# marbl/MHAP

Measured on AMD Instinct MI355X. Metric: overlaps/sec, higher is better.
Workload: dtype int64

## Files before the change

### include/mhap_hip.h

```cpp
#ifndef MHAP_HIP_H
#define MHAP_HIP_H

#include <stddef.h>
#include <stdint.h>

#ifdef __cplusplus
extern "C" {
#endif

#define MHAP_OK 0
#define MHAP_E_INVALID (-1)
#define MHAP_E_HIP (-2)
#define MHAP_E_NOMEM (-3)
#define MHAP_E_STATE (-4)
#define MHAP_E_IO (-5)

#define MHAP_STRAND_OK 0
#define MHAP_STRAND_ZERO_NGRAMS 1
#define MHAP_STRAND_TOO_SHORT 2

typedef struct mhap_params {
  int32_t kmer_size;
  int32_t num_hashes;
  int32_t ordered_kmer_size;
// ... 180 lines not shown

int mhap_align_pairs_banded(mhap_handle* h, const uint8_t* bases, int64_t n_bases, const int64_t* pairs , int64_t n,
                            int32_t* results );

int mhap_realign_plan(const mhap_record* recs, int64_t n, const int64_t* read_ids, const int64_t* offsets, const int32_t* lengths,
                      int64_t n_reads, double max_shift, int32_t band , int64_t* pairs );
const char* mhap_realign_plan_error(void);

int mhap_realign_records(mhap_handle* h, const uint8_t* bases, int64_t n_bases, const int64_t* read_ids, const int64_t* offsets,
                         const int32_t* lengths, int64_t n_reads, const mhap_record* recs, int64_t n, int32_t band,
                         mhap_record* out, int32_t* detail );

int mhap_pair_kmer_stats(mhap_handle* h, const uint8_t* bases, int64_t n_bases, const int64_t* pairs, int64_t n, int32_t k,
                         int32_t bottom_k, const uint8_t* skip, int64_t n_skip, int32_t* out, int32_t* paths);
void* mhap_ksim_dev_create(mhap_handle* h);
void mhap_ksim_dev_destroy(void* dev);
int mhap_ksim_dev_pair_stats(void* dev, const uint8_t* bases, int64_t n_bases, const int64_t* pairs, int64_t n, int32_t k, int32_t bottom_k,
                             const uint8_t* skip, int64_t n_skip, int32_t* out, int32_t* paths);
int mhap_ksim_dev_trials(void* dev, uint64_t seed, int64_t trial0, int64_t n, int32_t length, int32_t offset, double error_rate,
                         double ins_pct, double del_pct, double sub_pct, int32_t flags, const uint8_t* ref_bases,
                         const int64_t* ref_offsets, const int32_t* ref_lengths, int64_t n_ref, int32_t k, int32_t bottom_k,
                         const uint8_t* skip, int64_t n_skip, int32_t* stats, uint8_t* reads, int32_t* meta, int32_t* events,
                         int64_t* failed_trial);
int mhap_pair_kmer_stats_paths(const int64_t* pairs, int64_t n, int32_t k, int64_t lds_bytes, int32_t hashed, int32_t* path);

#define MHAP_KSIM_ONE_SIDED 1
#define MHAP_KSIM_SIM_ONLY 2
void* mhap_ksim_create(int64_t seed, int32_t length, int32_t offset, double error_rate, double ins_pct, double del_pct, double sub_pct,
                       int32_t flags, const uint8_t* ref_bases, const int64_t* ref_offsets, const int32_t* ref_lengths, int64_t n_ref);
int64_t mhap_ksim_next(void* state, int64_t n_trials, uint8_t* reads, int32_t* meta);
const char* mhap_ksim_error(void* state, int32_t* role);
void mhap_ksim_destroy(void* state);

int mhap_synth_reads(uint64_t seed, int64_t n, int32_t len, double coverage, double error_rate, char* bases);
int mhap_synth_reads_shard(uint64_t seed, int64_t n, int32_t len, double coverage, double error_rate, int64_t shard,
                           int64_t nshards, char* bases);
int mhap_synth_reads_repeats(uint64_t seed, int64_t n, int32_t len, double coverage, double error_rate, int64_t shard,
                             int64_t nshards, int32_t rep_len, int32_t rep_spacing, double rep_div, char* bases);
int mhap_synth_reads_genome(uint64_t seed, const uint8_t* genome, int64_t G, int64_t n, const int32_t* lengths, const int64_t* offsets,
                            double error_rate, char* bases);

int mhap_synth_truth(uint64_t seed, int64_t n, int32_t len, double coverage, int64_t G, const int32_t* lengths, double error_rate,
                     int64_t shard, int64_t nshards, int64_t* start, int64_t* span, int8_t* strand, int32_t* n_ins, int32_t* n_del,
                     int32_t* n_sub);

int mhap_histogram_stats(const int32_t* vals, const int64_t* numbers, int64_t n, double percent, double* mean, double* stdev, int64_t* cut);

int mhap_hash_kmer(const char* kmer, int32_t len, int32_t do_rc, int64_t* out);

int mhap_selftest_hash_windows(const char* seq, int32_t len, int32_t k, int32_t k2, int64_t* out64, int32_t* out32);
int mhap_selftest_bloom(const int64_t* hashes, int64_t n, int64_t size_bloom, const int64_t* probes, int64_t np, uint8_t* out_flags,
                        int64_t* out2);
int mhap_selftest_transpose32(uint32_t* a32);
int mhap_selftest_pass_min(int32_t S, int32_t k2, double threshold, double* scores, int32_t* pass_min);
int mhap_selftest_xorshift_jump(uint64_t key, int32_t nsteps, uint64_t* out);
int mhap_selftest_xorshift_unjump(uint64_t x, int32_t nsteps, uint64_t* out);
int mhap_selftest_kmer_windows(const char* seq, int32_t len, int32_t k, int32_t canonical, uint64_t* out, uint8_t* valid);
int mhap_selftest_overlap_lane(const int32_t* A, int32_t nA, int32_t lenA, const int32_t* B, int32_t nB, int32_t lenB,
                               double max_shift, int32_t stride, int32_t* out8);

#ifdef __cplusplus
}
#endif
#endif
```

### mhap_amd/api.py

```python
import ctypes as C
import os

import numpy as np

_HERE = os.path.dirname(os.path.abspath(__file__))
_LIB_PATH = os.environ.get("MHAP_LIB_PATH") or os.path.join(_HERE, "lib", "libmhaphip.so")
_lib = None

KERNEL_NAMES = ["hash_kmers", "kmer_weight", "minhash", "ordered", "candidate", "overlap", "index_build", "index_query"]


class MhapError(RuntimeError):
    """MhapRuntimeException analogue (J/impl/MhapRuntimeException.java:32)."""


class _Params(C.Structure):
    _fields_ = [("kmer_size", C.c_int32), ("num_hashes", C.c_int32), ("ordered_kmer_size", C.c_int32),
                ("ordered_sketch_size", C.c_int32), ("num_min_matches", C.c_int32), ("min_store_length", C.c_int32),
                ("min_olap_length", C.c_int32), ("device", C.c_int32), ("threshold", C.c_double),
                ("max_shift", C.c_double), ("repeat_weight", C.c_double)]


class _Stats(C.Structure):
    _fields_ = [("strands_indexed", C.c_int64), ("queries_searched", C.c_int64), ("candidates_compared", C.c_int64),
                ("matches_found", C.c_int64), ("slot_compares", C.c_int64), ("table_elements", C.c_int64),
                ("slow_pairs", C.c_int64), ("index_splits", C.c_int64)]


class _KTimes(C.Structure):
    _fields_ = [("ms", C.c_double * 8), ("launches", C.c_int64 * 8)]


class _Fasta(C.Structure):
    _fields_ = [("bases", C.c_void_p), ("offsets", C.c_void_p), ("lengths", C.c_void_p), ("ids", C.c_void_p),
                ("n", C.c_int64), ("total_bases", C.c_int64), ("headers", C.c_void_p), ("headers_bytes", C.c_int64)]


RECORD_DTYPE = np.dtype([("from_id", "<i8"), ("to_id", "<i8"), ("score", "<f8"), ("raw", "<f8"), ("a1", "<i4"),
                         ("a2", "<i4"), ("alen", "<i4"), ("b1", "<i4"), ("b2", "<i4"), ("blen", "<i4"),
                         ("to_rc", "<i4"), ("pad", "<i4")])
_SINK = C.CFUNCTYPE(C.c_int, C.c_void_p, C.c_int64, C.c_void_p)
_GATE = C.CFUNCTYPE(C.c_int, C.c_void_p)

EXPORTED_SYMBOLS = [
    "mhap_create", "mhap_destroy", "mhap_last_error", "mhap_default_params", "mhap_set_filter", "mhap_index_add_reads",
    "mhap_sketch_batch", "mhap_index_add_sketches", "mhap_index_size", "mhap_index_export", "mhap_index_clear", "mhap_index_prepare",
    "mhap_sketch_reads_device", "mhap_index_set_device", "mhap_find_matches_self", "mhap_find_matches_reads",
    "mhap_get_stats", "mhap_get_kernel_times", "mhap_reset_kernel_times", "mhap_set_stream", "mhap_synchronize",
    "mhap_format_record", "mhap_fasta_read", "mhap_fasta_free", "mhap_synth_reads", "mhap_hash_kmer",
    "mhap_selftest_hash_windows", "mhap_selftest_overlap_lane", "mhap_stage_reads", "mhap_index_add_staged",
    "mhap_sketch_staged_device", "mhap_find_matches_self_shard", "mhap_synth_reads_shard", "mhap_selftest_transpose32", "mhap_selftest_pass_min", "mhap_selftest_xorshift_jump", "mhap_selftest_xorshift_unjump", "mhap_find_matches_sketches",
    "mhap_synth_reads_repeats", "mhap_synth_reads_genome", "mhap_find_matches_device", "mhap_set_filter_whitelist", "mhap_set_filter_file", "mhap_selftest_bloom", "mhap_set_second_stage_gate",
    "mhap_dist_unique_id", "mhap_dist_init", "mhap_dist_finalize", "mhap_dist_find_matches_self", "mhap_dist_find_matches_reads", "mhap_dist_last_timing", "mhap_dist_exchange_timing", "mhap_dist_info", "mhap_dist_selftest", "mhap_dist_set_eager", "mhap_dist_eager_searches",
    "mhap_group_create", "mhap_group_destroy", "mhap_group_size", "mhap_group_rank", "mhap_group_last_error", "mhap_group_add_reads", "mhap_group_clear",
    "mhap_group_find_matches_self", "mhap_group_find_matches_reads", "mhap_group_get_stats", "mhap_abi_version", "mhap_abi_sizes",
    "mhap_index_reserve", "mhap_fasta_scan_open", "mhap_fasta_scan_free", "mhap_fasta_scan_reads", "mhap_fasta_scan_bases", "mhap_fasta_scan_info",
    "mhap_index_add_scan", "mhap_find_matches_scan", "mhap_group_add_scan",
    "mhap_kmer_count_begin", "mhap_kmer_count_add_reads", "mhap_kmer_count_add_scan", "mhap_kmer_count_finish", "mhap_kmer_counts_info",
    "mhap_kmer_counts_lines", "mhap_kmer_counts_write", "mhap_kmer_counts_free", "mhap_selftest_kmer_windows",
    "mhap_kmer_count_finish_flags", "mhap_kmer_counts_histogram_size", "mhap_kmer_counts_histogram", "mhap_kmer_counts_write_histogram",
    "mhap_histogram_stats",
    "mhap_synth_truth", "mhap_align_pairs",
    "mhap_align_pairs_banded", "mhap_realign_plan", "mhap_realign_plan_error", "mhap_realign_records",
    "mhap_pair_kmer_stats", "mhap_pair_kmer_stats_paths", "mhap_ksim_create", "mhap_ksim_next", "mhap_ksim_error", "mhap_ksim_destroy",
    "mhap_ksim_dev_create", "mhap_ksim_dev_destroy", "mhap_ksim_dev_pair_stats", "mhap_ksim_dev_trials",
]
MHAP_KMER_HISTOGRAM = 1
ABI_VERSION = 3


def load_library(build_if_missing=True):
    global _lib
    if _lib is not None:
        return _lib
    if not os.path.exists(_LIB_PATH):
        if not build_if_missing:
            raise MhapError(f"{_LIB_PATH} is missing: run `python -m mhap_amd.build`")
        from . import build as _b
        _b.build()
    try:
        import torch
    except Exception:
        pass
    try:
        lib = C.CDLL(_LIB_PATH)
    except OSError as e:
        raise MhapError(f"cannot load the HIP extension {_LIB_PATH}: {e}") from e
    lib.mhap_last_error.restype = C.c_char_p
    lib.mhap_last_error.argtypes = [C.c_void_p]
    lib.mhap_destroy.restype = None
    lib.mhap_destroy.argtypes = [C.c_void_p]
    lib.mhap_fasta_free.restype = None
    lib.mhap_default_params.restype = None
    lib.mhap_group_destroy.restype = None
    lib.mhap_group_destroy.argtypes = [C.c_void_p]
    lib.mhap_group_rank.restype = C.c_void_p
    lib.mhap_group_rank.argtypes = [C.c_void_p, C.c_int32]
    lib.mhap_group_last_error.restype = C.c_char_p
    lib.mhap_group_last_error.argtypes = [C.c_void_p]
    lib.mhap_group_size.argtypes = [C.c_void_p]
    lib.mhap_fasta_scan_free.restype = None
    lib.mhap_fasta_scan_free.argtypes = [C.c_void_p]
    lib.mhap_fasta_scan_reads.restype = C.c_int64
    lib.mhap_fasta_scan_reads.argtypes = [C.c_void_p]
    lib.mhap_fasta_scan_bases.restype = C.c_int64
    lib.mhap_fasta_scan_bases.argtypes = [C.c_void_p]
    lib.mhap_kmer_counts_free.restype = None
    lib.mhap_kmer_counts_free.argtypes = [C.c_void_p]
    for name, nargs in (("mhap_kmer_counts_info", 4), ("mhap_kmer_counts_lines", 2), ("mhap_kmer_counts_write", 1),
                        ("mhap_kmer_counts_histogram_size", 1), ("mhap_kmer_counts_histogram", 2), ("mhap_kmer_counts_write_histogram", 1)):
        getattr(lib, name).argtypes = [C.c_void_p] + [C.c_void_p] * nargs
    lib.mhap_histogram_stats.argtypes = [C.c_void_p, C.c_void_p, C.c_int64, C.c_double, C.c_void_p, C.c_void_p, C.c_void_p]
    lib.mhap_ksim_create.restype = C.c_void_p
    lib.mhap_ksim_create.argtypes = [C.c_int64, C.c_int32, C.c_int32, C.c_double, C.c_double, C.c_double, C.c_double, C.c_int32,
                                     C.c_void_p, C.c_void_p, C.c_void_p, C.c_int64]
    lib.mhap_ksim_next.restype = C.c_int64
    lib.mhap_ksim_next.argtypes = [C.c_void_p, C.c_int64, C.c_void_p, C.c_void_p]
    lib.mhap_ksim_error.restype = C.c_char_p
# ... 888 lines not shown
```

### mhap_amd/csrc/kernels.hpp

```cpp
#pragma once
#include "device_common.hpp"

namespace mhap {

constexpr int HASH_TILE = 1024;
constexpr int WEIGHT_THREADS = 1024;
constexpr int WEIGHT_MAXIT = 24;
constexpr int MH_U = 4;
constexpr int ORD_THREADS = 256;
constexpr int ORD_BINS = 2048;
constexpr int CAND_TQ = 128;
constexpr int CAND_TM = 128;
constexpr int CAND_KS = 32;
constexpr int OVL_THREADS = 128;
#ifndef MH_INV_CT
#define MH_INV_CT 2048
#endif
constexpr int INV_CT = MH_INV_CT;

constexpr int BS_WCLASSES = 6;
constexpr int BS_WMAX = 32;
struct StrandInfo { int32_t valid; int32_t mode; int32_t cnt[BS_WCLASSES + 1]; int32_t pad; };

struct FilterTable {
  const int64_t* keys;
  const double* vals;
  uint32_t mask;
  uint32_t size;
  int32_t enabled;
  int32_t no_tf;
  double range;
  const unsigned long long* bloom; uint64_t bloom_bits; int32_t bloom_k; int32_t bloom_mode;
};

constexpr int META_W = 4;

struct Candidate { int32_t q; int32_t m; };

struct DevRecord { int32_t q, m; double score; int32_t raw, a1, a2, b1, b2, pad; };

struct SearchParams {
  int32_t H, S, k2;
  int32_t num_min_matches, min_store_length;
  int32_t to_self;
  int32_t own_queries;
  double max_shift, threshold;
};

void launch_hash_kmers(hipStream_t st, const ReadDesc* descs, int64_t nstrands, int max_len, const uint8_t* store, int64_t* keys,
                       int32_t* h32, int k, int k2, const uint64_t* luts, int only_mat);
void build_kmer_hash_luts(uint64_t* out);
int weight_grid(int num_cus, int64_t nstrands, int max_len, int k);
bool strand_hashes_from_codes(int length, int k, int k2);
void launch_kmer_weights(hipStream_t st, int num_cus, const ReadDesc* descs, int64_t nstrands, int max_len, const int64_t* keys,
                         uint32_t* wts, uint32_t* perm, uint32_t* slabs, int64_t slab_entries, unsigned long long* counter, int k,
                         const FilterTable& ft, double repeat_weight, StrandInfo* info, bool fused, const uint8_t* store,
                         const uint64_t* luts, const int32_t* order, int32_t* slist);
bool launch_minhash(hipStream_t st, hipStream_t st_weighted, int nblocks, int64_t n_unweighted, int64_t n_weighted, const ReadDesc* descs, int64_t nstrands, const int64_t* keys, const uint32_t* wts,
                    const uint32_t* perm, const StrandInfo* info, const uint8_t* store, const uint64_t* luts, int k, int k2, int H,
                    unsigned long long* counter, int32_t* out_rows, int64_t out_stride, int32_t* out_status, int64_t status_stride,
                    const uint64_t* jump, int jump_na, const int32_t* slist, uint32_t* qbuf, const uint64_t* unjump, const uint64_t* jump_w1, unsigned long long* merge,
                    int max_nk);
size_t minhash_merge_bytes(int nblocks, int H);
void build_xorshift_unjump_tables(int na, int nq, uint64_t* out);
int minhash_wgs_per_cu(int H);
size_t minhash_queue_bytes(int nblocks_total, int H);
int minhash_queue_words(int H);
constexpr int XS_JUMP_LOG2 = 2;
constexpr int XS_JUMP_NQ = BS_WMAX;
#ifndef MH_W1_JUMP_NA
#define MH_W1_JUMP_NA 16
#endif
constexpr int W1_JUMP_NA = MH_W1_JUMP_NA;
inline int w1_jump_tables(int H) { return W1_JUMP_NA + ((H + 1) >> XS_JUMP_LOG2) / W1_JUMP_NA + 1; }
void build_xorshift_jump_tables(int na, int nq, uint64_t* out);
void launch_fix_status(hipStream_t st, int32_t* meta, int64_t nreads);
size_t ordered_lds_bytes(int cap, int code_words, int stage_wide);
void launch_ordered(hipStream_t st, const ReadDesc* descs, int64_t nstrands, int max_len_codes, int max_len, const int32_t* h32,
                    const uint8_t* store, const uint64_t* luts, int k2, int S, int cap, int32_t* out_rows, int64_t out_stride,
                    int32_t* out_meta, int64_t meta_stride, int64_t first = 0, int64_t count = -1);

void launch_candidates(hipStream_t st, const int32_t* minhash, int64_t row_stride, const int32_t* qminhash, int64_t qrow_stride,
                       const int32_t* qlist, int nq, int ne, const int64_t* ids, const int64_t* qids, const int32_t* meta,
                       const int32_t* qmeta, const SearchParams& sp, const long long* rowstart, long long nblocks_tri, Candidate* cand,
                       unsigned long long* cand_count, unsigned long long cand_cap);
constexpr int MHAP_MAX_NUM_HASHES = 8192;
int minhash_waves_per_workgroup(int H);
struct InvIndex {
  uint32_t* ends;
  uint2* items;
  uint32_t nb, shift;
  uint64_t slot_stride;
  uint32_t ne;
  uint32_t grouped;
  uint32_t group_t, class_log;
  uint32_t* lines;
  uint32_t nl_log, line_lb, line_ebits;
  uint32_t tile_entries, tiles;
  uint2* staged;
  uint32_t* tile_counts;
  uint32_t* bin_start;
  uint32_t* bin_long;
};
void launch_query_iota(hipStream_t st, int32_t* qlist, int first, int n);
int index_tile_entries(int ne);
void index_group_params(int64_t entries, InvIndex& ix);
int index_coarse_bins();
bool index_line_params(int64_t entries, uint32_t nb, uint32_t& nl_log, uint32_t& lb, uint32_t& ebits);
size_t index_line_bytes(int H, uint32_t nl_log);
int index_max_buckets_log();
void launch_index_verify(hipStream_t st, const int32_t* minhash, int64_t row_stride, const int32_t* meta, int ne, int H, const InvIndex& ix,
                         unsigned long long* missing);
bool launch_index_build(hipStream_t st, const int32_t* minhash, int64_t row_stride, const int32_t* meta, int ne, int H, const InvIndex& ix);
void launch_index_query(hipStream_t st, const InvIndex& ix, const int32_t* qminhash, int64_t qrow_stride,
                        const int32_t* qlist, int nq, const int64_t* ids, const int64_t* qids, const int32_t* meta, const int32_t* qmeta,
                        const SearchParams& sp, Candidate* cand, unsigned long long* cand_count, unsigned long long cand_cap,
                        unsigned long long* split_count, unsigned long long* elements_total, int32_t* big, unsigned long long* big_count, int tier,
                        unsigned long long* elements_spread);
int index_elements_spread_words();
int index_query_dense_ranges(int64_t entries);
bool index_query_tiers();
bool index_query_tier_ok(int tier, int64_t entries, int num_min_matches);
void oj_stats_dump();
void launch_overlap(hipStream_t st, int nblocks, const Candidate* cand, const unsigned long long* cand_count, unsigned long long cand_cap,
                    const int32_t* ordered, int64_t ord_stride, const int32_t* meta, const int32_t* qordered, int64_t qord_stride,
                    const int32_t* qmeta, const SearchParams& sp, const double* score_table, int32_t* scratch, int64_t scratch_per_lane,
                    DevRecord* recs, unsigned long long* rec_count, unsigned long long rec_cap, unsigned long long* compared, int spread);
size_t overlap_join_wide_lds_bytes(int S, int shape);
int overlap_join_wide_blocks_per_cu(int S, int shape);
int overlap_join_wide_waves_per_block(int shape);
// ... 31 lines not shown
```

### mhap_amd/csrc/mhap_capi.hip

```cpp
#include <algorithm>
#include <atomic>
#include <cmath>
#include <cstdio>
#include <cstdlib>
#include <chrono>
#include <cstring>
#include <condition_variable>
#include <functional>
#include <mutex>
#include <string>
#include <thread>
#include <vector>

#include "../../include/mhap_hip.h"
static double hp_now() { return std::chrono::duration<double, std::milli>(std::chrono::steady_clock::now().time_since_epoch()).count(); }
#define HPROF(tag) do { if (getenv("MHAP_HOST_PROF")) fprintf(stderr, "[host] %-28s %.3f ms\n", tag, hp_now()); } while (0)
#define DBGSYNC(h, tag) do { if (getenv("MHAP_DEBUG_SYNC")) { fprintf(stderr, "[dbg] %s launched\n", tag); hipError_t _e = hipStreamSynchronize((h)->stream); fprintf(stderr, "[dbg] %s done: %s\n", tag, hipGetErrorString(_e)); } } while (0)
#include "kernels.hpp"
#include "mhap_internal.hpp"
#include "overlap_lane.hpp"

using namespace mhap;

namespace {
// ... 1633 lines not shown
    for (int i = 0; i < 8; i++) y ^= T[i * 256 + (int)((x >> (8 * i)) & 255u)];
    x = y;
  }
  for (int t = 0; t < r; t++) x = xorshift_step(x);
  *out = x;
  return MHAP_OK;
}

int mhap_selftest_xorshift_unjump(uint64_t x, int32_t nsteps, uint64_t* out) {
  if (!out || nsteps < 1 || nsteps > (1 << 15)) return MHAP_E_INVALID;
  int a = (nsteps + (1 << XS_JUMP_LOG2) - 1) >> XS_JUMP_LOG2;
  const int r = (a << XS_JUMP_LOG2) - nsteps;
  const int qa = a > W1_JUMP_NA ? (a - 1) / W1_JUMP_NA : 0;
  a -= qa * W1_JUMP_NA;
  std::vector<uint64_t> ut((size_t)(W1_JUMP_NA + qa) * 2048);
  build_xorshift_unjump_tables(W1_JUMP_NA, qa, ut.data());
  uint64_t y = x;
  if (qa > 0) {
    const uint64_t* T = ut.data() + (size_t)(W1_JUMP_NA + qa - 1) * 2048;
    uint64_t z = 0;
    for (int i = 0; i < 8; i++) z ^= T[i * 256 + (int)((y >> (8 * i)) & 255u)];
    y = z;
  }
  {
    const uint64_t* T = ut.data() + (size_t)(a - 1) * 2048;
    uint64_t z = 0;
    for (int i = 0; i < 8; i++) z ^= T[i * 256 + (int)((y >> (8 * i)) & 255u)];
    y = z;
  }
  for (int t = 0; t < r; t++) y = xorshift_step(y);
  *out = y;
  return MHAP_OK;
}

int mhap_selftest_bloom(const int64_t* hashes, int64_t n, int64_t size_bloom, const int64_t* probes, int64_t np, uint8_t* out_flags, int64_t* out2) {
  if ((n > 0 && !hashes) || (np > 0 && (!probes || !out_flags)) || !out2) return MHAP_E_INVALID;
  std::vector<unsigned long long> words; uint64_t bit_size = 0; int k = 0;
  build_bloom(hashes, n, size_bloom, words, bit_size, k);
  for (int64_t i = 0; i < np; i++) out_flags[i] = bloom_might_contain(words.data(), bit_size, k, (uint64_t)probes[i]) ? 1 : 0;
  out2[0] = (int64_t)bit_size; out2[1] = k;
  return MHAP_OK;
}

int mhap_selftest_pass_min(int32_t S, int32_t k2, double threshold, double* scores, int32_t* pass_min) {
  if (S < 1 || S > 8192 || k2 < 1 || !pass_min) return MHAP_E_INVALID;
  std::vector<double> tbl; std::vector<int32_t> pm;
  fill_score_table(S, k2, tbl);
  build_pass_min(tbl, S, threshold, pm);
  if (scores) memcpy(scores, tbl.data(), tbl.size() * 8);
  memcpy(pass_min, pm.data(), pm.size() * 4);
  return MHAP_OK;
}

int mhap_selftest_transpose32(uint32_t* a32) {
  if (!a32) return MHAP_E_INVALID;
  uint32_t a[32];
  memcpy(a, a32, sizeof a);
  transpose32(a);
  memcpy(a32, a, sizeof a);
  return MHAP_OK;
}

int mhap_selftest_overlap_lane(const int32_t* A, int32_t nA, int32_t lenA, const int32_t* B, int32_t nB, int32_t lenB, double max_shift,
                               int32_t stride, int32_t* out8) {
  if (!A || !B || !out8 || stride < 1) return MHAP_E_INVALID;
  const int maxrec = 2 * std::max(nA, nB) + 2;
  std::vector<int32_t> scratch((size_t)3 * (size_t)maxrec * (size_t)stride, 0);
  LaneScratch sc; sc.base = scratch.data(); sc.stride = stride; sc.maxrec = maxrec;
  PlainView va{A, nA}, vb{B, nB};
  const LaneOverlap r = lane_overlap(va, lenA, vb, lenB, max_shift, sc);
  out8[0] = r.empty; out8[1] = r.valid; out8[2] = r.a1; out8[3] = r.a2; out8[4] = r.b1; out8[5] = r.b2; out8[6] = r.inter; out8[7] = r.kk;
  return MHAP_OK;
}

}

namespace mhap {
int internal_find_matches_device(mhap_handle* h, const void* d_q_minhash, const void* d_q_ordered, const void* d_q_meta, const int64_t* ids,
                                 const int64_t* d_ids_dev, int64_t m, int to_self, mhap_record_sink sink, void* user) {
  return find_matches_device_impl(h, d_q_minhash, d_q_ordered, d_q_meta, ids, d_ids_dev, m, to_self, sink, user);
}
}
```

### mhap_amd/csrc/sketch_kernels.hip

```cpp
#include <cstdlib>
#include <cstring>

#include "kernels.hpp"
#include <algorithm>

namespace mhap {

constexpr int HASH_SEG = 4096;
constexpr int HASH_LUT_WORDS = 3 * 256;

void build_kmer_hash_luts(uint64_t* out) {
  const uint64_t c1 = 0x87c37b91114253d5ULL, c2 = 0x4cf5ad432745937fULL;
  const uint32_t d1 = 0xcc9e2d51U, d2 = 0x1b873593U;
  const char* acgt = "ACGT";
  for (int idx = 0; idx < 256; idx++) {
    uint64_t block = 0;
    for (int c = 0; c < 4; c++) block |= (uint64_t)(uint8_t)acgt[(idx >> (2 * c)) & 3] << (16 * c);
    uint64_t k1 = block * c1; k1 = rotl64(k1, 31); k1 *= c2;
    uint64_t k2 = block * c2; k2 = rotl64(k2, 33); k2 *= c1;
    uint32_t a = (uint32_t)block, b = (uint32_t)(block >> 32);
    a *= d1; a = rotl32(a, 15); a *= d2;
    b *= d1; b = rotl32(b, 15); b *= d2;
    out[idx] = k1; out[256 + idx] = k2; out[512 + idx] = (uint64_t)a | ((uint64_t)b << 32);
  }
// ... 1792 lines not shown
      if (a.n_tail > 0) (void)hipMemsetAsync(merge, 0xFF, (size_t)a.n_tail * (size_t)H * 8, st);
      a.prof = nullptr;
      if (profmode) {
        static unsigned long long* dprof1 = nullptr;
        if (!dprof1) (void)hipMalloc(&dprof1, 8 * sizeof(unsigned long long));
        (void)hipMemsetAsync(dprof1, 0, 8 * sizeof(unsigned long long), st);
        a.prof = dprof1;
        static hipEvent_t pe0 = nullptr, pe1 = nullptr;
        if (!pe0) { (void)hipEventCreate(&pe0); (void)hipEventCreate(&pe1); }
        (void)hipEventRecord(pe0, st);
        if (qcap == BS_QCAP) hipLaunchKernelGGL((minhash_w1_kernel<true, true>), dim3(nb), dim3(256), lds1, st, a);
        else hipLaunchKernelGGL((minhash_w1_kernel<true, false>), dim3(nb), dim3(256), lds1, st, a);
        (void)hipEventRecord(pe1, st);
        unsigned long long hp[8];
        (void)hipMemcpyAsync(hp, dprof1, sizeof(hp), hipMemcpyDeviceToHost, st);
        (void)hipStreamSynchronize(st);
        const double tot = (double)hp[7];
        float pms = 0.f; (void)hipEventElapsedTime(&pms, pe0, pe1);
        fprintf(stderr, "[minhash w1 prof] launch %.3f ms, %d waves: mean shader clock %.0f MHz (wave-clocks / waves / time)\n", pms, nb * 4,
                pms > 0.f ? tot / ((double)nb * 4.0) / ((double)pms * 1e3) : 0.0);
        fprintf(stderr, "[minhash w1 prof] rows %llu (first-type %llu)  wave-clocks: total %.3g  key load+transpose %.1f%%  first-row slots %.1f%% (%.0f clocks/step)  "
                        "later-row slots %.1f%% (%.0f clocks/step)  drains %.1f%%  candidates/row %.0f\n", hp[4], hp[5], tot, 100.0 * hp[0] / tot, 100.0 * hp[1] / tot,
                hp[5] ? (double)hp[1] / ((double)hp[5] * H) : 0.0, 100.0 * hp[2] / tot, hp[4] > hp[5] ? (double)hp[2] / ((double)(hp[4] - hp[5]) * H) : 0.0,
                100.0 * hp[3] / tot, hp[4] ? (double)hp[6] / (double)hp[4] : 0.0);
      } else
        if (qcap == BS_QCAP) hipLaunchKernelGGL((minhash_w1_kernel<false, true>), dim3(nb), dim3(256), lds1, st, a);
        else hipLaunchKernelGGL((minhash_w1_kernel<false, false>), dim3(nb), dim3(256), lds1, st, a);
      if (a.n_tail > 0)
        hipLaunchKernelGGL(minhash_w1_finish_kernel, dim3((unsigned)((a.n_tail * (long long)H + 255) / 256)), dim3(256), 0, st, a);
      if (witness) snprintf(w1_path, sizeof(w1_path), "w1 n_whole %lld n_tail %lld rmax %d stagger %d", (long long)a.n_whole, (long long)a.n_tail, a.rmax, a.stagger);
    }
    if (witness)
      fprintf(stderr, "[minhash] strands %lld weight-1 %lld weighted %lld nblocks %d: weight-1 launch %s; weighted launch %s\n", (long long)nstrands,
              (long long)n_unweighted, (long long)n_weighted, nblocks, w1_path, nb_w > 0 ? (split ? "split" : "wave") : "none");
    return nb_w > 0;
  }
}


#ifdef MH_ORD_PROF
__device__ unsigned long long g_ord_prof[8];
#define ORD_TICK(k) do { __syncthreads(); if (threadIdx.x == 0) { const unsigned long long t_ = wall_clock64(); atomicAdd(&g_ord_prof[k], t_ - ord_t0); ord_t0 = t_; } } while (0)
#else
#define ORD_TICK(k) do { } while (0)
#endif
__device__ __forceinline__ uint32_t mm3_mul5c(uint32_t h) {
  uint32_t t;
  asm("v_lshl_add_u32 %0, %1, 2, %1" : "=v"(t) : "v"(h));
  return t + 0xe6546b64U;
}
constexpr uint32_t ORD_BUCKET_MAX = 32;
__device__ inline uint64_t okey(int32_t h, int pos) { return ((uint64_t)((uint32_t)h ^ 0x80000000u) << 32) | (uint32_t)pos; }

__global__ __launch_bounds__(ORD_THREADS) void ordered_kernel(const ReadDesc* __restrict__ descs, int64_t nstrands,
                                                              const int32_t* __restrict__ h32, const uint8_t* __restrict__ store,
                                                              const uint64_t* __restrict__ luts, int code_words, int stage_wide, int k2, int S, int cap,
                                                              int32_t* __restrict__ out_rows, int64_t out_stride,
                                                              int32_t* __restrict__ out_meta, int64_t meta_stride, int64_t first) {
  extern __shared__ __attribute__((aligned(16))) char smem[];
  uint32_t* hist = (uint32_t*)smem;
  uint32_t* part = hist + ORD_BINS;
  uint32_t* svars = part + ORD_THREADS;
  uint64_t* buf = (uint64_t*)(svars + 4);
  uint16_t* bstart = (uint16_t*)(buf + cap);
  uint32_t* stage = (uint32_t*)(bstart + ORD_BINS + 2);
  uint16_t* stage16 = (uint16_t*)stage;
  const size_t lut_off = ((size_t)ORD_BINS * 4 + (size_t)ORD_THREADS * 4 + 16 + (size_t)cap * 8 + (size_t)(ORD_BINS + 2) * 2 + (size_t)cap * (stage_wide ? 4 : 2) + 7) & ~(size_t)7;
  uint64_t* lut = (uint64_t*)(smem + lut_off);
  uint32_t* codes = (uint32_t*)(lut + 256);
  uint32_t& s_bin = svars[0]; uint32_t& s_below = svars[1]; uint32_t& s_cnt = svars[2]; uint32_t& s_fill = svars[3];
  const int64_t strand = first + (int64_t)blockIdx.x;
  if (strand >= nstrands) return;
#ifdef MH_ORD_PROF
  unsigned long long ord_t0 = wall_clock64();
#endif
  const ReadDesc rd = descs[strand >> 1];
  const int rcs = (int)(strand & 1);
  const int n = rd.length - k2 + 1;
  int32_t* meta = out_meta + strand * meta_stride;
  if (strand_skipped(rd, rcs) || n < 1) {
    if (threadIdx.x == 0) { meta[0] = 0; meta[1] = n; meta[2] = rd.length; }
    return;
  }
  const bool mat = (rd.flags & MHAP_RD_MAT) != 0;
  const int32_t* hp = h32 + rd.h2_off + (rcs ? rd.h2_stride : 0);
  if (!mat) {
    for (int i = threadIdx.x; i < 256; i += ORD_THREADS) lut[i] = luts[512 + i];
    const int ncw = (rd.length + 15) / 16 + 2;
    for (int wj = threadIdx.x; wj < ncw && wj < code_words; wj += ORD_THREADS) codes[wj] = strand_codes16(store + rd.base_off, rd.length, rcs, 16 * wj);
    __syncthreads();
  }
  ORD_TICK(0);
  auto hget = [&](int i) -> int32_t {
    if (mat) return hp[i];
    const uint32_t cw = codes_at(codes, i);
    uint32_t h = 0;
#pragma unroll
    for (int q = 0; q < 3; q++) {
      const uint64_t kk = lut[(cw >> (8 * q)) & 255u];
      h ^= (uint32_t)kk;         h = rotl32(h, 13); h = mm3_mul5c(h);
      h ^= (uint32_t)(kk >> 32); h = rotl32(h, 13); h = mm3_mul5c(h);
    }
    h ^= 24u;
    return (int32_t)fmix32(h);
  };
  const int K = S < n ? S : n;
  if (threadIdx.x == 0) { meta[0] = K; meta[1] = n; meta[2] = rd.length; }
// ... 227 lines not shown
    }
    __syncthreads();
    int32_t* orow = out_rows + strand * out_stride;
    for (uint32_t t = threadIdx.x; t < bk_total; t += ORD_THREADS) {
      const uint64_t key = buf[t];
      const uint32_t b = (uint32_t)(key >> 53), s0 = bstart[b], c = hist[b];
      uint32_t rank = 0;
      for (uint32_t q = 0; q < c; q += 4) {
        uint64_t o[4];
#pragma unroll
        for (int x = 0; x < 4; x++) o[x] = buf[s0 + q + (uint32_t)x < (uint32_t)cap ? s0 + q + (uint32_t)x : s0];
#pragma unroll
        for (int x = 0; x < 4; x++) rank += (q + (uint32_t)x < c && o[x] < key) ? 1u : 0u;
      }
      const uint32_t j = s0 + rank;
      if (j < (uint32_t)K) { orow[2 * j] = (int32_t)((uint32_t)(key >> 32) ^ 0x80000000u); orow[2 * j + 1] = (int32_t)(uint32_t)key; }
    }
    return;
  }
  __syncthreads();
  for (int i = threadIdx.x; i < n; i += ORD_THREADS) {
    const uint64_t key = okey(hget(i), i);
    if (key <= bound) { uint32_t slot = atomicAdd(&s_fill, 1u); if (slot < (uint32_t)cap) buf[slot] = key; }
  }
  __syncthreads();
  const uint32_t m = s_fill < (uint32_t)cap ? s_fill : (uint32_t)cap;
  uint32_t np2 = 1;
  while (np2 < m) np2 <<= 1;
  for (uint32_t j = m + threadIdx.x; j < np2; j += ORD_THREADS) buf[j] = ~0ULL;
  __syncthreads();
  for (uint32_t size = 2; size <= np2; size <<= 1) {
    for (uint32_t stride = size >> 1; stride > 0; stride >>= 1) {
      for (uint32_t t = threadIdx.x; t < (np2 >> 1); t += ORD_THREADS) {
        const uint32_t lo = 2 * t - (t & (stride - 1));
        const uint32_t hi = lo + stride;
        const bool up = ((lo & size) == 0);
        const uint64_t a = buf[lo], b = buf[hi];
        if ((a > b) == up) { buf[lo] = b; buf[hi] = a; }
      }
      __syncthreads();
    }
  }
  int32_t* orow = out_rows + strand * out_stride;
  for (int j = threadIdx.x; j < K; j += ORD_THREADS) {
    const uint64_t key = buf[j];
    orow[2 * j] = (int32_t)((uint32_t)(key >> 32) ^ 0x80000000u);
    orow[2 * j + 1] = (int32_t)(uint32_t)key;
  }
}

#ifndef MH_ORD_PAD
#define MH_ORD_PAD 0
#endif
size_t ordered_lds_bytes(int cap, int code_words, int stage_wide) {
  return (size_t)ORD_BINS * 4 + (size_t)ORD_THREADS * 4 + 16 + (size_t)cap * 8 + (size_t)(ORD_BINS + 2) * 2 + (size_t)cap * (stage_wide ? 4 : 2) +
         (code_words > 0 ? (size_t)256 * 8 + (size_t)code_words * 4 : 0) + 8 + MH_ORD_PAD;
}

__global__ void fix_status_kernel(int32_t* __restrict__ meta, int64_t nreads) {
  const int64_t i = (int64_t)blockIdx.x * blockDim.x + threadIdx.x;
  if (i >= nreads) return;
  const int32_t fs = meta[(2 * i) * META_W + 3];
  if (fs != 0 && meta[(2 * i + 1) * META_W + 3] == 0) meta[(2 * i + 1) * META_W + 3] = fs;
}

void launch_fix_status(hipStream_t st, int32_t* meta, int64_t nreads) {
  if (nreads <= 0) return;
  hipLaunchKernelGGL(fix_status_kernel, dim3((unsigned)((nreads + 255) / 256)), dim3(256), 0, st, meta, nreads);
}

void launch_ordered(hipStream_t st, const ReadDesc* descs, int64_t nstrands, int max_len_codes, int max_len, const int32_t* h32,
                    const uint8_t* store, const uint64_t* luts, int k2, int S, int cap, int32_t* out_rows, int64_t out_stride,
                    int32_t* out_meta, int64_t meta_stride, int64_t first, int64_t count) {
  if (count < 0 || first + count > nstrands) count = nstrands - first;
  if (nstrands <= 0 || count <= 0) return;
  const int code_words = max_len_codes > 0 ? (max_len_codes + 15) / 16 + 4 : 0;
  const int stage_wide = max_len - k2 + 1 > 65535 ? 1 : 0;
  hipLaunchKernelGGL(ordered_kernel, dim3((unsigned)count), dim3(ORD_THREADS), ordered_lds_bytes(cap, code_words, stage_wide), st, descs, nstrands, h32,
                     store, luts, code_words, stage_wide, k2, S, cap, out_rows, out_stride, out_meta, meta_stride, first);
#ifdef MH_ORD_PROF
  (void)hipStreamSynchronize(st);
  unsigned long long hp[8];
  (void)hipMemcpyFromSymbol(hp, HIP_SYMBOL(g_ord_prof), sizeof(hp));
  fprintf(stderr, "[ordered prof] cap %d lds %zu strands(one-pass) %llu  100MHz ticks/strand: stage %.1f pass1 %.1f scan %.1f fill %.1f isort %.1f out %.1f\n", cap,
          ordered_lds_bytes(cap, code_words, stage_wide), hp[7], (double)hp[0] / hp[7], (double)hp[1] / hp[7], (double)hp[2] / hp[7], (double)hp[3] / hp[7],
          (double)hp[4] / hp[7], (double)hp[5] / hp[7]);
  unsigned long long z[8] = {0, 0, 0, 0, 0, 0, 0, 0};
  (void)hipMemcpyToSymbol(HIP_SYMBOL(g_ord_prof), z, sizeof(z));
#endif
}

}
```

Baseline: 459,200.

## Replace ordered-sketch kernel with lower-LDS counting-sort and rank-based selection

Adds a new ordered_kernel that keeps bucket counts as packed 16-bit pairs and overlays the histogram on the key buffer and the permutation array on the LUT region. This cuts LDS per workgroup so more workgroups fit per CU. It replaces the per-bucket insertion sort with a direct rank computation within each bucket, and writes output as 8-byte pairs when alignment allows. The old kernel stays available behind an environment variable, and optional path counters and an occupancy report are added, at the cost of more code and a narrower 16-bit count range.

Measured after the change: 458,900, median of 2. About the same (-0.1%).

```diff
diff --git a/include/mhap_hip.h b/include/mhap_hip.h
--- a/include/mhap_hip.h
+++ b/include/mhap_hip.h
@@ -256,6 +256,7 @@
 int mhap_selftest_bloom(const int64_t* hashes, int64_t n, int64_t size_bloom, const int64_t* probes, int64_t np, uint8_t* out_flags,
                         int64_t* out2);
 int mhap_selftest_transpose32(uint32_t* a32);
+int mhap_ordered_path_counts(uint64_t out[4], int32_t reset);
 int mhap_selftest_pass_min(int32_t S, int32_t k2, double threshold, double* scores, int32_t* pass_min);
 int mhap_selftest_xorshift_jump(uint64_t key, int32_t nsteps, uint64_t* out);
 int mhap_selftest_xorshift_unjump(uint64_t x, int32_t nsteps, uint64_t* out);
diff --git a/mhap_amd/api.py b/mhap_amd/api.py
--- a/mhap_amd/api.py
+++ b/mhap_amd/api.py
@@ -64,6 +64,7 @@
     "mhap_align_pairs_banded", "mhap_realign_plan", "mhap_realign_plan_error", "mhap_realign_records",
     "mhap_pair_kmer_stats", "mhap_pair_kmer_stats_paths", "mhap_ksim_create", "mhap_ksim_next", "mhap_ksim_error", "mhap_ksim_destroy",
     "mhap_ksim_dev_create", "mhap_ksim_dev_destroy", "mhap_ksim_dev_pair_stats", "mhap_ksim_dev_trials",
+    "mhap_ordered_path_counts",
 ]
 MHAP_KMER_HISTOGRAM = 1
 ABI_VERSION = 3
diff --git a/mhap_amd/csrc/kernels.hpp b/mhap_amd/csrc/kernels.hpp
--- a/mhap_amd/csrc/kernels.hpp
+++ b/mhap_amd/csrc/kernels.hpp
@@ -75,7 +75,9 @@
 inline int w1_jump_tables(int H) { return W1_JUMP_NA + ((H + 1) >> XS_JUMP_LOG2) / W1_JUMP_NA + 1; }
 void build_xorshift_jump_tables(int na, int nq, uint64_t* out);
 void launch_fix_status(hipStream_t st, int32_t* meta, int64_t nreads);
-size_t ordered_lds_bytes(int cap, int code_words, int stage_wide);
+size_t ordered_lds_bytes(int cap, int code_words);
+size_t ordered_lds_bytes_v1(int cap, int code_words, int stage_wide);
+void ordered_path_counts(unsigned long long out[4], bool reset);
 void launch_ordered(hipStream_t st, const ReadDesc* descs, int64_t nstrands, int max_len_codes, int max_len, const int32_t* h32,
                     const uint8_t* store, const uint64_t* luts, int k2, int S, int cap, int32_t* out_rows, int64_t out_stride,
                     int32_t* out_meta, int64_t meta_stride, int64_t first = 0, int64_t count = -1);
diff --git a/mhap_amd/csrc/mhap_capi.hip b/mhap_amd/csrc/mhap_capi.hip
--- a/mhap_amd/csrc/mhap_capi.hip
+++ b/mhap_amd/csrc/mhap_capi.hip
@@ -1709,6 +1709,14 @@
   return MHAP_OK;
 }
 
+int mhap_ordered_path_counts(uint64_t out[4], int32_t reset) {
+  if (!out) return MHAP_E_INVALID;
+  unsigned long long c[4] = {0, 0, 0, 0};
+  ordered_path_counts(c, reset != 0);
+  for (int i = 0; i < 4; i++) out[i] = c[i];
+  return MHAP_OK;
+}
+
 int mhap_selftest_transpose32(uint32_t* a32) {
   if (!a32) return MHAP_E_INVALID;
   uint32_t a[32];
diff --git a/mhap_amd/csrc/sketch_kernels.hip b/mhap_amd/csrc/sketch_kernels.hip
--- a/mhap_amd/csrc/sketch_kernels.hip
+++ b/mhap_amd/csrc/sketch_kernels.hip
@@ -1868,7 +1868,7 @@
 constexpr uint32_t ORD_BUCKET_MAX = 32;
 __device__ inline uint64_t okey(int32_t h, int pos) { return ((uint64_t)((uint32_t)h ^ 0x80000000u) << 32) | (uint32_t)pos; }
 
-__global__ __launch_bounds__(ORD_THREADS) void ordered_kernel(const ReadDesc* __restrict__ descs, int64_t nstrands,
+__global__ __launch_bounds__(ORD_THREADS) void ordered_kernel_v1(const ReadDesc* __restrict__ descs, int64_t nstrands,
                                                               const int32_t* __restrict__ h32, const uint8_t* __restrict__ store,
                                                               const uint64_t* __restrict__ luts, int code_words, int stage_wide, int k2, int S, int cap,
                                                               int32_t* __restrict__ out_rows, int64_t out_stride,
@@ -2202,9 +2202,357 @@
 #ifndef MH_ORD_PAD
 #define MH_ORD_PAD 0
 #endif
-size_t ordered_lds_bytes(int cap, int code_words, int stage_wide) {
+size_t ordered_lds_bytes_v1(int cap, int code_words, int stage_wide) {
   return (size_t)ORD_BINS * 4 + (size_t)ORD_THREADS * 4 + 16 + (size_t)cap * 8 + (size_t)(ORD_BINS + 2) * 2 + (size_t)cap * (stage_wide ? 4 : 2) +
          (code_words > 0 ? (size_t)256 * 8 + (size_t)code_words * 4 : 0) + 8 + MH_ORD_PAD;
+}
+
+__device__ unsigned long long g_ord_paths[4];
+__device__ __forceinline__ uint32_t ord_cw(uint32_t b) { return b & (uint32_t)(ORD_BINS / 2 - 1); }
+__device__ __forceinline__ uint32_t ord_cs(uint32_t b) { return (b / (uint32_t)(ORD_BINS / 2)) * 16u; }
+__device__ __forceinline__ uint32_t ord_ci(uint32_t b) { return 2u * ord_cw(b) + b / (uint32_t)(ORD_BINS / 2); }
+__device__ __forceinline__ void ord_store_pair(int32_t* __restrict__ orow, uint32_t j, uint64_t key, int pair8) {
+  const int32_t hh = (int32_t)((uint32_t)(key >> 32) ^ 0x80000000u), pp = (int32_t)(uint32_t)key;
+  if (pair8) ((int2*)orow)[j] = make_int2(hh, pp);
+  else { orow[2 * j] = hh; orow[2 * j + 1] = pp; }
+}
+template <bool IND>
+__device__ __forceinline__ void ord_rank_write(const uint64_t* buf, const uint16_t* perm, const uint16_t* c16, uint32_t m, uint32_t K, int32_t* __restrict__ orow, int pair8) {
+  for (uint32_t t0 = threadIdx.x; t0 < m; t0 += 2 * ORD_THREADS) {
+    uint64_t key[2]; uint32_t s0[2], c[2], rank[2] = {0u, 0u};
+#pragma unroll
+    for (int u = 0; u < 2; u++) {
+      const uint32_t t = t0 + (uint32_t)u * ORD_THREADS;
+      key[u] = buf[t < m ? t : t0];
+      const uint32_t b = (uint32_t)(key[u] >> 53);
+      s0[u] = b ? (uint32_t)c16[ord_ci(b - 1)] : 0u;
+      c[u] = t < m ? (uint32_t)c16[ord_ci(b)] - s0[u] : 0u;
+    }
+    const uint32_t cmax = c[0] > c[1] ? c[0] : c[1];
+    for (uint32_t q = 0; q < cmax; q += 4) {
+      uint32_t ix[2][4]; uint64_t o[2][4];
+#pragma unroll
+      for (int u = 0; u < 2; u++)
+#pragma unroll
+        for (int x = 0; x < 4; x++) { const uint32_t sl = s0[u] + q + (uint32_t)x < m ? s0[u] + q + (uint32_t)x : s0[u]; ix[u][x] = IND ? (uint32_t)perm[sl] : sl; }
+#pragma unroll
+      for (int u = 0; u < 2; u++)
+#pragma unroll
+        for (int x = 0; x < 4; x++) o[u][x] = buf[ix[u][x]];
+#pragma unroll
+      for (int u = 0; u < 2; u++)
+#pragma unroll
+        for (int x = 0; x < 4; x++) rank[u] += (q + (uint32_t)x < c[u] && o[u][x] < key[u]) ? 1u : 0u;
+    }
+#pragma unroll
+    for (int u = 0; u < 2; u++) {
+      const uint32_t j = s0[u] + rank[u];
+      if (t0 + (uint32_t)u * ORD_THREADS < m && j < K) ord_store_pair(orow, j, key[u], pair8);
+    }
+  }
+}
+
+__global__ __launch_bounds__(ORD_THREADS) void ordered_kernel(const ReadDesc* __restrict__ descs, int64_t nstrands,
+                                                              const int32_t* __restrict__ h32, const uint8_t* __restrict__ store,
+                                                              const uint64_t* __restrict__ luts, int code_words, int k2, int S, int cap,
+                                                              int32_t* __restrict__ out_rows, int64_t out_stride,
+                                                              int32_t* __restrict__ out_meta, int64_t meta_stride, int64_t first, int pair8, int stats) {
+  extern __shared__ __attribute__((aligned(16))) char smem[];
+  uint32_t* cnt = (uint32_t*)smem;
+  uint16_t* c16 = (uint16_t*)smem;
+  uint32_t* svars = cnt + ORD_BINS / 2 + 2;
+  uint32_t* part = svars + 4;
+  uint64_t* buf = (uint64_t*)(svars + 8);
+  uint32_t* hist = (uint32_t*)buf;
+  const size_t buf_bytes = (size_t)cap * 8 > (size_t)ORD_BINS * 4 ? (size_t)cap * 8 : (size_t)ORD_BINS * 4;
+  const size_t lut_off = (size_t)(ORD_BINS / 2 + 2) * 4 + 32 + buf_bytes;
+  uint64_t* lut = (uint64_t*)(smem + lut_off);
+  uint32_t* codes = (uint32_t*)(lut + 256);
+  uint16_t* perm = (uint16_t*)(smem + lut_off);
+  uint32_t& s_bin = svars[0]; uint32_t& s_below = svars[1]; uint32_t& s_cnt = svars[2]; uint32_t& s_fill = svars[3];
+  const int64_t strand = first + (int64_t)blockIdx.x;
+  if (strand >= nstrands) return;
+#ifdef MH_ORD_PROF
+  unsigned long long ord_t0 = wall_clock64();
+#endif
+  const ReadDesc rd = descs[strand >> 1];
+  const int rcs = (int)(strand & 1);
+  const int n = rd.length - k2 + 1;
+  int32_t* meta = out_meta + strand * meta_stride;
+  if (strand_skipped(rd, rcs) || n < 1) {
+    if (threadIdx.x == 0) { meta[0] = 0; meta[1] = n; meta[2] = rd.length; }
+    return;
+  }
+  const bool mat = (rd.flags & MHAP_RD_MAT) != 0;
+  const int32_t* hp = h32 + rd.h2_off + (rcs ? rd.h2_stride : 0);
+  if (!mat) {
+    for (int i = threadIdx.x; i < 256; i += ORD_THREADS) lut[i] = luts[512 + i];
+    const int ncw = (rd.length + 15) / 16 + 2;
+    for (int wj = threadIdx.x; wj < ncw && wj < code_words; wj += ORD_THREADS) codes[wj] = strand_codes16(store + rd.base_off, rd.length, rcs, 16 * wj);
+    __syncthreads();
+  }
+  ORD_TICK(0);
+  auto hget = [&](int i) -> int32_t {
+    if (mat) return hp[i];
+    const uint32_t cw = codes_at(codes, i);
+    uint32_t h = 0;
+#pragma unroll
+    for (int q = 0; q < 3; q++) {
+      const uint64_t kk = lut[(cw >> (8 * q)) & 255u];
+      h ^= (uint32_t)kk;         h = rotl32(h, 13); h = mm3_mul5c(h);
+      h ^= (uint32_t)(kk >> 32); h = rotl32(h, 13); h = mm3_mul5c(h);
+    }
+    h ^= 24u;
+    return (int32_t)fmix32(h);
+  };
+  const int K = S < n ? S : n;
+  if (threadIdx.x == 0) { meta[0] = K; meta[1] = n; meta[2] = rd.length; }
+  if (K <= 0) return;
+  int32_t* orow = out_rows + strand * out_stride;
+
+  const double ksig = sqrt((double)K), csig = sqrt((double)cap);
+  const double target = fmin((double)K + 7.0 * ksig, (double)cap - 5.0 * csig);
+  if (n > cap && target >= (double)K + 3.0 * ksig) {
+    const double quant = target / (double)n;
+    const uint32_t cut_u = quant >= 1.0 ? 0xFFFFFFFFu : (uint32_t)(quant * 4294967296.0);
+    for (uint32_t j = threadIdx.x; j < ORD_BINS / 2 + 2; j += ORD_THREADS) cnt[j] = 0;
+    if (threadIdx.x == 0) { s_fill = 0; s_cnt = 0; }
+    __syncthreads();
+    const int lane = threadIdx.x & 63;
+    for (int ib = 0; ib < n; ib += 8 * ORD_THREADS) {
+      const int p0 = ib + 32 * (int)(threadIdx.x >> 2) + (int)(threadIdx.x & 3);
+      int32_t hv[8];
+      if (mat) {
+#pragma unroll
+        for (int u = 0; u < 8; u++) { const int i = p0 + 4 * u; hv[u] = i < n ? hp[i] : 0; }
+      } else if (p0 < n) {
+        const int d = p0 >> 4;
+        const uint32_t sh = (uint32_t)(2 * (p0 & 15));
+        const uint32_t w0 = codes[d], w1 = codes[d + 1], w2 = codes[d + 2], w3 = codes[d + 3];
+        const uint32_t a[3] = {__builtin_amdgcn_alignbit(w1, w0, sh), __builtin_amdgcn_alignbit(w2, w1, sh), __builtin_amdgcn_alignbit(w3, w2, sh)};
+        uint64_t g[10];
+#pragma unroll
+        for (int j = 0; j < 10; j++) g[j] = lut[(a[j >> 2] >> (8 * (j & 3))) & 255u];
+#pragma unroll
+        for (int u = 0; u < 8; u++) {
+          uint32_t h = 0;
+#pragma unroll
+          for (int q = 0; q < 3; q++) {
+            const uint64_t kk = g[u + q];
+            h ^= (uint32_t)kk;         h = rotl32(h, 13); h = mm3_mul5c(h);
+            h ^= (uint32_t)(kk >> 32); h = rotl32(h, 13); h = mm3_mul5c(h);
+          }
+          h ^= 24u;
+          hv[u] = (int32_t)fmix32(h);
+        }
+      } else {
+#pragma unroll
+        for (int u = 0; u < 8; u++) hv[u] = 0;
+      }
+      unsigned long long bal[8];
+      uint32_t total = 0;
+#pragma unroll
+      for (int u = 0; u < 8; u++) {
+        bal[u] = __ballot(p0 + 4 * u < n && ((uint32_t)hv[u] ^ 0x80000000u) < cut_u);
+        total += (uint32_t)__popcll(bal[u]);
+      }
+      if (total) {
+        uint32_t base = 0;
+        if (lane == 0) base = atomicAdd(&s_fill, total);
+        base = (uint32_t)__builtin_amdgcn_readfirstlane((int)base);
+#pragma unroll
+        for (int u = 0; u < 8; u++) {
+          if ((bal[u] >> lane) & 1ULL) {
+            const uint32_t idx = base + __builtin_amdgcn_mbcnt_hi((uint32_t)(bal[u] >> 32), __builtin_amdgcn_mbcnt_lo((uint32_t)bal[u], 0u));
+            const uint32_t b = ((uint32_t)hv[u] ^ 0x80000000u) >> 21;
+            if (idx < (uint32_t)cap) buf[idx] = okey(hv[u], p0 + 4 * u);
+            atomicAdd(&cnt[ord_cw(b)], 1u << ord_cs(b));
+          }
+          base += (uint32_t)__popcll(bal[u]);
+        }
+      }
+    }
+    __syncthreads();
+    ORD_TICK(1);
+    const uint32_t m = s_fill;
+    bool ok = m >= (uint32_t)K && m <= (uint32_t)cap;
+    if (ok) {
+      constexpr int per = ORD_BINS / ORD_THREADS;
+      uint32_t cj[per];
+      uint32_t loc = 0, mx = 0;
+#pragma unroll
+      for (int j = 0; j < per; j++) { cj[j] = c16[ord_ci(threadIdx.x * per + j)]; loc += cj[j]; mx = cj[j] > mx ? cj[j] : mx; }
+      uint32_t incl = loc;
+#pragma unroll
+      for (int off = 1; off < 64; off <<= 1) { const uint32_t v = __shfl_up(incl, off); if (lane >= off) incl += v; }
+      if (lane == 63) part[threadIdx.x >> 6] = incl;
+      if (mx > ORD_BUCKET_MAX) atomicMax(&s_cnt, mx);
+      __syncthreads();
+      for (unsigned w = 0; w < (threadIdx.x >> 6); w++) incl += part[w];
+      ok = s_cnt == 0;
+      if (ok) {
+        uint32_t run = incl - loc;
+#pragma unroll
+        for (int j = 0; j < per; j++) { c16[ord_ci(threadIdx.x * per + j)] = (uint16_t)run; run += cj[j]; }
+      }
+      __syncthreads();
+    }
+    ORD_TICK(2);
+    if (ok) {
+      for (uint32_t t0 = threadIdx.x; t0 < m; t0 += 4 * ORD_THREADS) {
+        uint32_t b[4], old[4];
+#pragma unroll
+        for (int u = 0; u < 4; u++) { const uint32_t t = t0 + (uint32_t)u * ORD_THREADS; b[u] = (uint32_t)(buf[t < m ? t : t0] >> 53); }
+#pragma unroll
+        for (int u = 0; u < 4; u++) old[u] = t0 + (uint32_t)u * ORD_THREADS < m ? atomicAdd(&cnt[ord_cw(b[u])], 1u << ord_cs(b[u])) : 0u;
+#pragma unroll
+        for (int u = 0; u < 4; u++) if (t0 + (uint32_t)u * ORD_THREADS < m) perm[(old[u] >> ord_cs(b[u])) & 0xFFFFu] = (uint16_t)(t0 + (uint32_t)u * ORD_THREADS);
+      }
+      __syncthreads();
+      ORD_TICK(3);
+      ord_rank_write<true>(buf, perm, c16, m, (uint32_t)K, orow, pair8);
+      ORD_TICK(5);
+#ifdef MH_ORD_PROF
+      if (threadIdx.x == 0) atomicAdd(&g_ord_prof[7], 1ULL);
+#endif
+      if (stats && threadIdx.x == 0) atomicAdd(&g_ord_paths[0], 1ULL);
+      return;
+    }
+    if (stats && threadIdx.x == 0) atomicAdd(&g_ord_paths[3], 1ULL);
+    __syncthreads();
+  }
+
+  uint64_t bound = ~0ULL;
+  bool buckets = false;
+  uint32_t bk_bin = 0, bk_total = 0;
+  if (threadIdx.x == 0) s_fill = 0;
+  if (n > cap) {
+    const int shifts[6] = {53, 42, 32, 21, 10, 0};
+    const int widths[6] = {11, 11, 10, 11, 11, 10};
+    uint64_t prefix = 0;
+    uint64_t prefmask = 0;
+    uint32_t below = 0;
+    for (int lv = 0; lv < 6; lv++) {
+      const int sh = shifts[lv];
+      const uint32_t nb = 1u << widths[lv];
+      for (uint32_t j = threadIdx.x; j < ORD_BINS; j += ORD_THREADS) hist[j] = 0;
+      __syncthreads();
+      for (int i0 = threadIdx.x; i0 < n; i0 += 8 * ORD_THREADS) {
+        int32_t hv[8];
+#pragma unroll
+        for (int u = 0; u < 8; u++) { const int i = i0 + u * ORD_THREADS; hv[u] = i < n ? hget(i) : 0; }
+#pragma unroll
+        for (int u = 0; u < 8; u++) {
+          const int i = i0 + u * ORD_THREADS;
+          const uint64_t key = okey(hv[u], i);
+          if (i < n && (key & prefmask) == prefix) atomicAdd(&hist[(uint32_t)(key >> sh) & (nb - 1)], 1u);
+        }
+      }
+      __syncthreads();
+      const uint32_t target = (uint32_t)(K - 1) - below;
+      const int per = ORD_BINS / ORD_THREADS;
+      uint32_t loc = 0;
+      for (int j = 0; j < per; j++) loc += hist[threadIdx.x * per + j];
+      uint32_t incl = loc;
+#pragma unroll
+      for (int off = 1; off < 64; off <<= 1) {
+        const uint32_t v = __shfl_up(incl, off);
+        if ((threadIdx.x & 63) >= (unsigned)off) incl += v;
+      }
+      if ((threadIdx.x & 63) == 63) part[threadIdx.x >> 6] = incl;
+      __syncthreads();
+      for (unsigned w = 0; w < (threadIdx.x >> 6); w++) incl += part[w];
+      const uint32_t excl = incl - loc;
+      if (target >= excl && target < incl) {
+        uint32_t run = excl;
+        for (int j = 0; j < per; j++) {
+          const uint32_t c = hist[threadIdx.x * per + j];
+          if (target < run + c) { s_bin = threadIdx.x * per + j; s_below = run; s_cnt = c; break; }
+          run += c;
+        }
+      }
+      __syncthreads();
+      const uint32_t bin = s_bin, binbelow = s_below, bincnt = s_cnt;
+      __syncthreads();
+      below += binbelow;
+      prefix |= (uint64_t)bin << sh;
+      prefmask |= (uint64_t)(nb - 1) << sh;
+      bound = prefix | (sh > 0 ? ((1ULL << sh) - 1) : 0ULL);
+      if (below + bincnt <= (uint32_t)cap) {
+        if (lv == 0) {
+          uint32_t run = excl, mx = 0;
+          for (int j = 0; j < per; j++) {
+            const uint32_t b = threadIdx.x * per + j, c = hist[b];
+            if (b <= bin) { c16[ord_ci(b)] = (uint16_t)run; mx = c > mx ? c : mx; }
+            run += c;
+          }
+          if (mx > ORD_BUCKET_MAX) atomicMax(&s_fill, mx);
+          __syncthreads();
+          buckets = s_fill == 0;
+          bk_bin = bin; bk_total = below + bincnt;
+          __syncthreads();
+          if (threadIdx.x == 0) s_fill = 0;
+        }
+        break;
+      }
+    }
+  }
+  if (buckets) {
+    __syncthreads();
+    for (int i0 = threadIdx.x; i0 < n; i0 += 8 * ORD_THREADS) {
+      int32_t hv[8];
+#pragma unroll
+      for (int u = 0; u < 8; u++) { const int i = i0 + u * ORD_THREADS; hv[u] = i < n ? hget(i) : 0; }
+#pragma unroll
+      for (int u = 0; u < 8; u++) {
+        const int i = i0 + u * ORD_THREADS;
+        const uint64_t key = okey(hv[u], i);
+        const uint32_t b = (uint32_t)(key >> 53);
+        if (i < n && b <= bk_bin) buf[(atomicAdd(&cnt[ord_cw(b)], 1u << ord_cs(b)) >> ord_cs(b)) & 0xFFFFu] = key;
+      }
+    }
+    __syncthreads();
+    ord_rank_write<false>(buf, nullptr, c16, bk_total, (uint32_t)K, orow, pair8);
+    if (stats && threadIdx.x == 0) atomicAdd(&g_ord_paths[1], 1ULL);
+    return;
+  }
+  __syncthreads();
+  for (int i = threadIdx.x; i < n; i += ORD_THREADS) {
+    const uint64_t key = okey(hget(i), i);
+    if (key <= bound) { uint32_t slot = atomicAdd(&s_fill, 1u); if (slot < (uint32_t)cap) buf[slot] = key; }
+  }
+  __syncthreads();
+  const uint32_t m = s_fill < (uint32_t)cap ? s_fill : (uint32_t)cap;
+  uint32_t np2 = 1;
+  while (np2 < m) np2 <<= 1;
+  for (uint32_t j = m + threadIdx.x; j < np2; j += ORD_THREADS) buf[j] = ~0ULL;
+  __syncthreads();
+  for (uint32_t size = 2; size <= np2; size <<= 1) {
+    for (uint32_t stride = size >> 1; stride > 0; stride >>= 1) {
+      for (uint32_t t = threadIdx.x; t < (np2 >> 1); t += ORD_THREADS) {
+        const uint32_t lo = 2 * t - (t & (stride - 1));
+        const uint32_t hi = lo + stride;
+        const bool up = ((lo & size) == 0);
+        const uint64_t a = buf[lo], b = buf[hi];
+        if ((a > b) == up) { buf[lo] = b; buf[hi] = a; }
+      }
+      __syncthreads();
+    }
+  }
+  for (int j = threadIdx.x; j < K; j += ORD_THREADS) ord_store_pair(orow, (uint32_t)j, buf[j], pair8);
+  if (stats && threadIdx.x == 0) atomicAdd(&g_ord_paths[2], 1ULL);
+}
+
+size_t ordered_lds_bytes(int cap, int code_words) {
+  const size_t buf_bytes = (size_t)cap * 8 > (size_t)ORD_BINS * 4 ? (size_t)cap * 8 : (size_t)ORD_BINS * 4;
+  const size_t tab = code_words > 0 ? (size_t)256 * 8 + (size_t)code_words * 4 : 0, perm = (size_t)cap * 2;
+  return (size_t)(ORD_BINS / 2 + 2) * 4 + 32 + buf_bytes + (tab > perm ? tab : perm) + 8 + MH_ORD_PAD;
+}
+
+void ordered_path_counts(unsigned long long out[4], bool reset) {
+  (void)hipDeviceSynchronize();
+  (void)hipMemcpyFromSymbol(out, HIP_SYMBOL(g_ord_paths), 4 * sizeof(unsigned long long));
+  if (reset) { const unsigned long long z[4] = {0, 0, 0, 0}; (void)hipMemcpyToSymbol(HIP_SYMBOL(g_ord_paths), z, sizeof(z)); }
 }
 
 __global__ void fix_status_kernel(int32_t* __restrict__ meta, int64_t nreads) {
@@ -2226,14 +2574,32 @@
   if (nstrands <= 0 || count <= 0) return;
   const int code_words = max_len_codes > 0 ? (max_len_codes + 15) / 16 + 4 : 0;
   const int stage_wide = max_len - k2 + 1 > 65535 ? 1 : 0;
-  hipLaunchKernelGGL(ordered_kernel, dim3((unsigned)count), dim3(ORD_THREADS), ordered_lds_bytes(cap, code_words, stage_wide), st, descs, nstrands, h32,
-                     store, luts, code_words, stage_wide, k2, S, cap, out_rows, out_stride, out_meta, meta_stride, first);
+  const bool v1 = []() { const char* e = getenv("MHAP_ORDERED_V1"); return e && atoi(e) != 0; }();
+  const int stats = []() { const char* e = getenv("MHAP_ORD_STATS"); return e && atoi(e) != 0 ? 1 : 0; }();
+  const size_t lds = v1 ? ordered_lds_bytes_v1(cap, code_words, stage_wide) : ordered_lds_bytes(cap, code_words);
+  if (const char* e = getenv("MHAP_ORD_OCC")) {
+    if (atoi(e) != 0) {
+      int wgs = 0;
+      const hipError_t oe = v1 ? hipOccupancyMaxActiveBlocksPerMultiprocessor(&wgs, ordered_kernel_v1, ORD_THREADS, lds)
+                               : hipOccupancyMaxActiveBlocksPerMultiprocessor(&wgs, ordered_kernel, ORD_THREADS, lds);
+      fprintf(stderr, "[ordered occ] kernel %s cap %d code_words %d: LDS %zu bytes per workgroup, %d workgroups resident per CU (%s)\n", v1 ? "v1" : "v2", cap,
+              code_words, lds, wgs, hipGetErrorString(oe));
+    }
+  }
+  if (v1)
+    hipLaunchKernelGGL(ordered_kernel_v1, dim3((unsigned)count), dim3(ORD_THREADS), lds, st, descs, nstrands, h32,
+                       store, luts, code_words, stage_wide, k2, S, cap, out_rows, out_stride, out_meta, meta_stride, first);
+  else {
+    const int pair8 = ((uintptr_t)out_rows & 7) == 0 && (out_stride & 1) == 0 ? 1 : 0;
+    hipLaunchKernelGGL(ordered_kernel, dim3((unsigned)count), dim3(ORD_THREADS), lds, st, descs, nstrands, h32,
+                       store, luts, code_words, k2, S, cap, out_rows, out_stride, out_meta, meta_stride, first, pair8, stats);
+  }
 #ifdef MH_ORD_PROF
   (void)hipStreamSynchronize(st);
   unsigned long long hp[8];
   (void)hipMemcpyFromSymbol(hp, HIP_SYMBOL(g_ord_prof), sizeof(hp));
   fprintf(stderr, "[ordered prof] cap %d lds %zu strands(one-pass) %llu  100MHz ticks/strand: stage %.1f pass1 %.1f scan %.1f fill %.1f isort %.1f out %.1f\n", cap,
-          ordered_lds_bytes(cap, code_words, stage_wide), hp[7], (double)hp[0] / hp[7], (double)hp[1] / hp[7], (double)hp[2] / hp[7], (double)hp[3] / hp[7],
+          lds, hp[7], (double)hp[0] / hp[7], (double)hp[1] / hp[7], (double)hp[2] / hp[7], (double)hp[3] / hp[7],
           (double)hp[4] / hp[7], (double)hp[5] / hp[7]);
   unsigned long long z[8] = {0, 0, 0, 0, 0, 0, 0, 0};
   (void)hipMemcpyToSymbol(HIP_SYMBOL(g_ord_prof), z, sizeof(z));
```
